# AlgoLab/rs-vgaligner

Measured on AMD Instinct MI355X. Metric: aligned reads/sec (10 kbp ONT vs HLA graph), higher is better.
Workload: dtype int32+f64

## Files before the change

### rs-vgaligner_amd/binding.py

```python
from __future__ import annotations

import ctypes as C
import os
from typing import List, Optional, Sequence

import numpy as np

_HERE = os.path.dirname(os.path.abspath(__file__))
LIB_PATH = os.environ.get("VGA_LIB") or os.path.join(_HERE, "libvga_hip.so")

VGA_OK = 0
VGA_MAX_KMER_LENGTH = 32
VGA_STRANDS_FORWARD = 0
VGA_STRANDS_BOTH = 1
ERR_NAMES = {-1: "VGA_ERR_ARG", -2: "VGA_ERR_HIP", -3: "VGA_ERR_NOMEM", -4: "VGA_ERR_UNSUPPORTED",
             -5: "VGA_ERR_NO_INDEX", -6: "VGA_ERR_NO_DEVICE", -7: "VGA_ERR_POOL"}

PILEUP_COLUMNS = ("A", "C", "G", "T", "N", "del", "ins")

ABI_SYMBOLS = [
    "vga_ctx_create", "vga_ctx_destroy", "vga_last_error", "vga_ctx_synchronize", "vga_abi_version",
    "vga_index_upload", "vga_batch_create", "vga_batch_destroy", "vga_batch_strands", "vga_map_default_params", "vga_map_batch",
    "vga_map_result_free", "vga_poa_default_params", "vga_poa_result_free", "vga_poa_batch", "vga_align_batch",
    "vga_align_result_free", "vga_last_kernel_times", "vga_chain_paths_text", "vga_chain_text_free",
    "vga_align_prepare", "vga_ctx_set_pool_fraction", "vga_ctx_set_host_threads",
    "vga_index_build_kmers", "vga_index_kmers_free",
    "vga_coverage_begin", "vga_coverage_read", "vga_coverage_reset", "vga_coverage_end",
    "vga_path_support_begin", "vga_path_support_read", "vga_path_support_last", "vga_path_support_reset", "vga_path_support_end",
    "vga_path_support_lists",
    "vga_pileup_begin", "vga_pileup_read", "vga_pileup_reset", "vga_pileup_end",
    "vga_genotype_begin", "vga_genotype_read", "vga_genotype_reset", "vga_genotype_end", "vga_genotype_pairs",
    "vga_genotype_lik_table", "vga_genotype_lik_begin", "vga_genotype_lik_read", "vga_genotype_lik_reset", "vga_genotype_lik_end",
    "vga_genotype_lik_pairs", "vga_genotype_lik_source",
    "vga_path_edit_begin", "vga_path_edit_read", "vga_path_edit_last", "vga_path_edit_reset", "vga_path_edit_end", "vga_path_edit_pairs",
    "vga_variant_call", "vga_variant_call_table",
    "vga_insertion_begin", "vga_insertion_read", "vga_insertion_reset", "vga_insertion_end", "vga_insertion_call", "vga_insertion_call_table",
    "vga_phase_begin", "vga_phase_read", "vga_phase_reset", "vga_phase_end", "vga_phase_links", "vga_phase_links_lists", "vga_phase_chain",
    "vga_phase_tags", "vga_phase_tags_lists",
    "vga_haplotype_counts", "vga_haplotype_counts_lists", "vga_haplotype_jobs", "vga_haplotype_call",
# ... 171 lines not shown
def load_library():
    global _lib
    if _lib is not None:
        return _lib
    if not os.path.exists(LIB_PATH):
        raise RuntimeError(f"{LIB_PATH} is missing: build it with `python -c 'import __graft_entry__ as g; g.build()'` "
                           "(there is no CPU fallback)")
    L = C.CDLL(LIB_PATH)
    vp = C.c_void_p
    L.vga_ctx_create.argtypes = [C.c_int, _P(vp)]
    L.vga_ctx_destroy.argtypes = [vp]
    L.vga_last_error.argtypes = [vp]
    L.vga_last_error.restype = C.c_char_p
    L.vga_ctx_synchronize.argtypes = [vp]
    L.vga_index_upload.argtypes = [vp, _P(IndexDesc)]
    L.vga_batch_create.argtypes = [vp, C.c_char_p, _P(C.c_uint64), C.c_uint64, _P(vp)]
    L.vga_batch_destroy.argtypes = [vp]
    if hasattr(L, "vga_batch_strands"):
        L.vga_batch_strands.argtypes = [vp, C.c_int, _P(C.c_char), _P(C.c_char)]
        L.vga_batch_strands.restype = C.c_int
    L.vga_map_default_params.argtypes = [_P(MapParams)]
    L.vga_map_batch.argtypes = [vp, _P(MapParams), _P(_P(MapResult))]
    L.vga_map_result_free.argtypes = [_P(MapResult)]
    L.vga_poa_default_params.argtypes = [_P(PoaParams)]
    L.vga_poa_result_free.argtypes = [_P(PoaResult)]
    L.vga_poa_batch.argtypes = [vp, C.c_uint64, _P(C.c_uint64), _P(C.c_uint64), C.c_char_p, _P(C.c_uint64),
                                _P(C.c_uint32), _P(C.c_uint32), _P(C.c_uint64), C.c_char_p, _P(PoaParams),
                                _P(_P(PoaResult))]
    L.vga_align_batch.argtypes = [vp, _P(MapResult), C.c_uint32, _P(PoaParams), _P(_P(AlignResult))]
    L.vga_align_result_free.argtypes = [_P(AlignResult)]
    L.vga_last_kernel_times.argtypes = [vp, _P(KernelTime), C.c_int]
    L.vga_chain_paths_text.argtypes = [vp, _P(MapResult), _P(_P(ChainText))]
    L.vga_align_prepare.argtypes = [vp, C.c_uint64, C.c_uint32]
    L.vga_align_prepare.restype = C.c_int
    L.vga_ctx_set_pool_fraction.argtypes = [vp, C.c_double]
    L.vga_ctx_set_pool_fraction.restype = C.c_int
    L.vga_ctx_set_host_threads.argtypes = [vp, C.c_uint32]
    L.vga_ctx_set_host_threads.restype = C.c_int
    L.vga_chain_text_free.argtypes = [_P(ChainText)]
    L.vga_index_build_kmers.argtypes = [vp, _P(IndexDesc), C.c_uint64, C.c_uint64]
    L.vga_index_build_kmers.restype = C.c_int
    L.vga_index_kmers_free.argtypes = [_P(IndexDesc)]
    L.vga_index_kmers_free.restype = None
    if hasattr(L, "vga_coverage_begin"):
        for name in ("vga_coverage_begin", "vga_coverage_reset", "vga_coverage_end"):
            getattr(L, name).argtypes = [vp]
# ... 305 lines not shown
        self.anchor_off = _np(r.anchor_off, R + 1, np.uint64)
        self.anchor_id = _np(r.anchor_id, A, np.uint32) if r.anchor_id else None
        self.query_begin = _np(r.query_begin, A, np.uint32)
        self.target_begin = _np(r.target_begin, A, np.uint32)
        self.target_end = _np(r.target_end, A, np.uint32)
        self.max_chain_score = _np(r.max_chain_score, A, np.float64) if r.max_chain_score else None
        self.best_pred_id = _np(r.best_pred_id, A, np.int32) if r.best_pred_id else None
        self.curr_max = _np(r.curr_max, R, np.float64)
        self.chain_off = _np(r.chain_off, R + 1, np.uint64)
        self.chain_placeholder = _np(r.chain_placeholder, nc, np.uint8)
        self.chain_anchor_off = _np(r.chain_anchor_off, nc + 1, np.uint64)
        self.chain_anchor_idx = _np(r.chain_anchor_idx, int(self.chain_anchor_off[-1]) if nc else 0, np.uint32)
        self.ms = {"probe": r.ms_probe, "sort": r.ms_sort, "chain": r.ms_chain, "total": r.ms_total}
        self.n_hits = int(r.n_hits)
        self.strand = _np(r.strand, R, np.uint8) if r.strand else None

    def chains_of(self, read: int):
        out = []
        for c in range(int(self.chain_off[read]), int(self.chain_off[read + 1])):
            s, e = int(self.chain_anchor_off[c]), int(self.chain_anchor_off[c + 1])
            out.append((bool(self.chain_placeholder[c]), self.chain_anchor_idx[s:e].tolist()))
        return out

    def close(self):
        if self._ptr is not None:
            self._L.vga_map_result_free(self._ptr)
            self._ptr = None

    def __del__(self):
        try:
            self.close()
        except Exception:
            pass


class PoaOut:
    def __init__(self, L, ptr):
        r = ptr.contents
        n = int(r.n)
        self.n = n
        self.ok = _np(r.ok, n, np.uint8)
        self.best_score = _np(r.best_score, n, np.int32)
        self.path_off = _np(r.path_off, n + 1, np.uint64)
        tp = int(self.path_off[-1])
        self.abpoa_nodes = _np(r.abpoa_nodes, tp, np.uint32)
        self.graph_nodes = _np(r.graph_nodes, tp, np.uint32)
        self.aln_start_offset = _np(r.aln_start_offset, n, np.uint32)
        self.aln_end_offset = _np(r.aln_end_offset, n, np.uint32)
        self.n_aligned_bases = _np(r.n_aligned_bases, n, np.uint32)
# ... 766 lines not shown
```

### rs-vgaligner_amd/csrc/vga_align.hip

```cpp
#include "vga_align_plan.hpp"
#include "vga_common.hpp"
#include "vga_coverage.hpp"
#include "vga_path_edit.hpp"
#include "vga_path_support.hpp"
#include "vga_pileup.hpp"
#include "vga_insertion.hpp"
#include "vga_poa_internal.hpp"
#include "vga_subgraph_host.hpp"

#include <algorithm>
#include <atomic>
#include <chrono>
#include <memory>

extern "C" void vga_align_result_free(vga_align_result *r)
{
    if (!r) return;
    free(r->aligned); free(r->path_off); free(r->path_handles); free(r->path_length); free(r->path_start);
    free(r->path_end); free(r->block_length); free(r->best_score); free(r->cigar_off); free(r->cigar);
    free(r->cs_off); free(r->cs);
    free(r);
}

namespace {
// ... 55 lines not shown
    if (m->strand)
        for (uint64_t r = 0; r < R && !any_rev; r++) any_rev = m->strand[r] != 0;
    if (!any_rev) return VGA_OK;
    const int rc = vga_batch_revcomp_device(b);
    if (rc != VGA_OK) return rc;
    vga_batch_revcomp_host(b);
    tr.mark("reverse complement");
    return VGA_OK;
}

int align_call::plan()
{
    const char *refused = nullptr;
    for (const oplist_maker *mk : oplist_makers()) {
        if (on_device || refused) break;
        refused = mk->counting(ctx) ? mk->text.refusal : mk == &cov_maker() && ps ? OPLIST_REFUSAL_PATHS : nullptr;
    }
    if (refused) return vga_set_error(ctx, VGA_ERR_UNSUPPORTED, OPLIST_ERR_REFUSED, refused);
    align_select(m, align_best_n, prob_read, prob_chain, read_prob0);
    n = prob_read.size();
    proxy.resize(n);
    west.resize(n);
    descs.resize(n);
    std::atomic<int> has_reverse{0};
    vga_parallel_for(n, [&](uint64_t p) {
        const align_prob a = align_plan_problem(m, prob_read[p], prob_chain[p], qlen(prob_read[p]), ctx->index.k, sw);
        proxy[p] = a.proxy; west[p] = a.west; descs[p] = a.desc;
        if (a.reverse) has_reverse = 1;
    });
    std::vector<uint32_t> ord(n);
    std::iota(ord.begin(), ord.end(), 0u);
    if (on_device) {
        ord = align_launch_order(proxy);
        align_permute(prob_read, ord); align_permute(prob_chain, ord); align_permute(proxy, ord); align_permute(west, ord); align_permute(descs, ord);
    }
    slot_of = align_slot_of(ord);
    if (has_reverse)
        return vga_set_error(ctx, VGA_ERR_UNSUPPORTED,
                             "a chain to be aligned holds reverse-strand anchors: RangeOrient::Reverse / Both (src/align.rs:365-387) is not supported");
    feed.views.resize(n);
    q_src.resize(on_device ? n : 0);
    for (uint64_t p = 0; p < n; p++) {
        const uint64_t r = prob_read[p];
        feed.views[p] = {nullptr, nullptr, 0, nullptr, nullptr, 0, b->reads.data() + q_off(r), qlen(r)};
        if (on_device) q_src[p] = q_off(r);
    }
    feed.proxy = proxy.data();
    return VGA_OK;
}

int align_call::device_store()
{
// ... 235 lines not shown
```

### rs-vgaligner_amd/csrc/vga_align_plan.hpp

```cpp
#pragma once

#include <algorithm>
#include <cmath>
#include <cstdint>
#include <cstdlib>
#include <cstring>
#include <numeric>
#include <vector>

#include "../../include/vga_hip.h"
#include "vga_sg_records.hpp"

struct align_switches {
    bool sg_host = false;
    uint32_t giant_rows = 24000u;
    double giant_cells = 1.5e8;
    bool has_sg_split = false;
    long sg_split = 0;
    bool trace = false;
};

static inline align_switches align_read_switches()
{
    align_switches s;
    if (const char *e = getenv("VGA_SUBGRAPH")) s.sg_host = strstr(e, "host") != nullptr;
    if (const char *e = getenv("VGA_GIANT_ROWS")) s.giant_rows = (uint32_t)atol(e);
    if (const char *e = getenv("VGA_GIANT_CELLS")) s.giant_cells = atof(e);
    if (const char *e = getenv("VGA_SG_SPLIT")) { s.has_sg_split = true; s.sg_split = atol(e); }
    if (const char *e = getenv("VGA_TRACE")) s.trace = atoi(e) != 0;
    return s;
}

static inline void align_select(const vga_map_result *m, uint32_t best_n, std::vector<uint64_t> &prob_read, std::vector<uint64_t> &prob_chain,
                                std::vector<uint64_t> &read_prob0)
{
    const uint64_t R = m->n_reads;
    prob_read.clear();
    prob_chain.clear();
    read_prob0.assign(R + 1, 0);
    for (uint64_t r = 0; r < R; r++) {
        read_prob0[r] = prob_read.size();
        const uint64_t c0 = m->chain_off[r], c1 = m->chain_off[r + 1];
        const uint64_t take = std::min<uint64_t>(best_n, c1 - c0);
        for (uint64_t c = c0; c < c0 + take; c++)
            if (!m->chain_placeholder[c]) { prob_read.push_back(r); prob_chain.push_back(c); }
    }
    read_prob0[R] = prob_read.size();
}

struct align_prob {
    sg_desc desc;
    uint32_t lo, hi;
    float west;
    double proxy;
    bool reverse;
};

static inline align_prob align_plan_problem(const vga_map_result *m, uint64_t r, uint64_t c, uint32_t qlen, uint32_t k, const align_switches &sw)
{
    align_prob o = {};
    const uint64_t a0 = m->anchor_off[r];
    const uint64_t c0 = m->chain_anchor_off[c], c1 = m->chain_anchor_off[c + 1];
    uint32_t lo = 0xFFFFFFFFu, hi = 0, pmin = 0xFFFFFFFFu, pmax = 0;
    for (uint64_t t = c0; t < c1; t++) {
        const uint64_t ai = a0 + m->chain_anchor_idx[t];
        lo = std::min(lo, m->target_begin[ai]);
        hi = std::max(hi, m->target_end[ai]);
        if ((m->target_begin[ai] | m->target_end[ai]) >> 31) o.reverse = true;
        const uint32_t s = m->target_begin[ai], e = m->target_end[ai] - 1;
        pmin = std::min(pmin, std::min(s, e));
        pmax = std::max(pmax, std::max(s, e));
    }
    o.lo = lo;
    o.hi = hi;
    const double q_first = c1 > c0 ? (double)m->query_begin[a0 + m->chain_anchor_idx[c0]] : 0.0;
    const double q_last = c1 > c0 ? (double)m->query_begin[a0 + m->chain_anchor_idx[c1 - 1]] + (double)k : (double)qlen;
    const double uncovered = q_first + std::max(0.0, (double)qlen - q_last);
    const double rows = (double)(hi > lo ? hi - lo : 0) + 1.6 * uncovered;
    o.west = (float)(650.0 + 0.3 * std::max(0.0, 0.85 * rows - (double)qlen));
    o.proxy = rows * (double)o.west;
    if (rows >= 0.85 * (double)sw.giant_rows) o.proxy += 1e13;
    if (c1 > c0) {
        const uint64_t fa = a0 + m->chain_anchor_idx[c0], la = a0 + m->chain_anchor_idx[c1 - 1];
        o.desc = {pmin, pmax, m->query_begin[fa], m->target_begin[fa], m->query_begin[la], m->target_end[la], qlen, 0u};
    }
    return o;
}

static inline std::vector<uint32_t> align_launch_order(const std::vector<double> &proxy)
{
    std::vector<uint32_t> ord(proxy.size());
    std::iota(ord.begin(), ord.end(), 0u);
    std::stable_sort(ord.begin(), ord.end(), [&](uint32_t x, uint32_t y) { return proxy[x] > proxy[y]; });
    return ord;
}

static inline std::vector<uint32_t> align_slot_of(const std::vector<uint32_t> &ord)
{
    std::vector<uint32_t> slot_of(ord.size());
    for (size_t i = 0; i < ord.size(); i++) slot_of[ord[i]] = (uint32_t)i;
    return slot_of;
}

template <typename T>
static inline void align_permute(std::vector<T> &v, const std::vector<uint32_t> &ord)
{
    std::vector<T> w(v.size());
    for (size_t i = 0; i < ord.size(); i++) w[i] = v[ord[i]];
    v.swap(w);
// ... 23 lines not shown
```

### rs-vgaligner_amd/csrc/vga_common.hpp

```cpp
#pragma once

#include <hip/hip_runtime.h>
#include <sys/mman.h>

#include <chrono>
#include <cstdarg>
#include <cstdint>
#include <cstdio>
#include <cstdlib>
#include <cstring>
#include <atomic>
#include <memory>
#include <mutex>
#include <new>
#include <string>
#include <thread>
#include <vector>

#include "../../include/vga_hip.h"
#include "vga_probe_hash.hpp"

#define VGA_ABI_VERSION 6

template <typename T>
using vga_owned = std::unique_ptr<T, void (*)(T *)>;
template <typename T, typename U = T>
vga_owned<T> vga_make_owned()
{
    return vga_owned<T>(new (std::nothrow) U(), [](T *p) { delete static_cast<U *>(p); });
}

struct cov_state;
struct ps_state;
struct pu_state;
struct ia_state;
struct ph_state;
struct poa_ws;

struct vga_dev_index {
    uint32_t k = 0;
    uint64_t seq_length = 0;
    uint64_t n_nodes = 0, n_edges = 0;
    uint32_t *d_table = nullptr;
// ... 38 lines not shown
    double pool_fraction = 1.0;
    unsigned host_threads = 0;
    std::mutex deferred_mu;
    std::vector<vga_deferred> deferred;
    std::atomic<int> alloc_urgent{0};
    vga_dev_index index;
    std::vector<vga_timer_entry> timers;
    std::vector<hipEvent_t> event_pool;
    size_t events_used = 0;
    struct agg_t {
        std::string name;
        float ms;
        uint32_t launches;
        uint64_t bytes;
        float busy_ms;
    };
    std::vector<agg_t> last_times;
    int n_cu = 256;
    vga_owned<void> map_ws{nullptr, nullptr};
    vga_owned<struct poa_ws> poa_ws{nullptr, nullptr};
    vga_owned<void> sg_ws{nullptr, nullptr};
    vga_owned<void> gaf_ws{nullptr, nullptr};
    std::vector<struct vga_batch *> batches;
};

struct vga_batch {
    vga_ctx *ctx = nullptr;
    int device = 0;
    uint64_t n_reads = 0;
    uint64_t total_bases = 0;
    std::vector<uint64_t> read_off;
    std::vector<char> reads;
    char *d_reads = nullptr;
    uint64_t *d_read_off = nullptr;
    bool rc_dev = false, rc_host = false;
    uint64_t *d_read_off2 = nullptr;
};
int vga_batch_revcomp_device(vga_batch *b);
void vga_batch_revcomp_host(vga_batch *b);

int vga_set_error(vga_ctx *ctx, int code, const char *fmt, ...);
void vga_index_release(vga_dev_index &ix);
int vga_index_load_graph(vga_ctx *ctx, const vga_index_desc *d);

#define VGA_HIP_CHECK(ctx, call)                                                               \
    do {                                                                                       \
        hipError_t e_ = (call);                                                                \
// ... 173 lines not shown
```

### rs-vgaligner_amd/csrc/vga_ctx.hip

```cpp
#include "vga_common.hpp"

#include <mutex>

#include <algorithm>

#include <malloc.h>

int vga_set_error(vga_ctx *ctx, int code, const char *fmt, ...)
{
    char buf[1024];
    va_list ap;
    va_start(ap, fmt);
    vsnprintf(buf, sizeof buf, fmt, ap);
    va_end(ap);
    if (ctx) { std::lock_guard<std::mutex> lk(ctx->err_mu); ctx->err = buf; }
    return code;
}

unsigned vga_host_threads(uint64_t n)
{
    unsigned nt = std::thread::hardware_concurrency();
    if (nt == 0) nt = 4;
    if (nt > 32) nt = 32;
    const char *e = getenv("VGA_HOST_THREADS");
// ... 25 lines not shown
void vga_defer_release(void *device_ptr, void *pinned_ptr, void *registered_ptr, size_t registered_bytes)
{
    const vga_deferred d = {device_ptr, pinned_ptr, registered_ptr, registered_bytes};
    vga_ctx *ctx = t_current_ctx;
    if (!ctx) { release_one(d); return; }
    std::lock_guard<std::mutex> lk(ctx->deferred_mu);
    ctx->deferred.push_back(d);
}

void vga_release_deferred(vga_ctx *ctx)
{
    if (!ctx) return;
    std::vector<vga_deferred> todo;
    {
        std::lock_guard<std::mutex> lk(ctx->deferred_mu);
        todo.swap(ctx->deferred);
    }
    if (todo.empty()) return;
    int cur = 0;
    (void)hipGetDevice(&cur);
    if (cur != ctx->device) (void)hipSetDevice(ctx->device);
    for (const vga_deferred &d : todo) release_one(d);
    if (cur != ctx->device) (void)hipSetDevice(cur);
}

extern "C" int vga_ctx_set_pool_fraction(vga_ctx *ctx, double fraction)
{
    if (!ctx) return VGA_ERR_ARG;
    if (!(fraction > 0.0) || fraction > 1.0) return vga_set_error(ctx, VGA_ERR_ARG, "vga_ctx_set_pool_fraction: %g is not in (0, 1]", fraction);
    ctx->pool_fraction = fraction;
    return VGA_OK;
}

extern "C" int vga_ctx_set_host_threads(vga_ctx *ctx, uint32_t n_threads)
{
    if (!ctx) return VGA_ERR_ARG;
    if (n_threads > 1024) return vga_set_error(ctx, VGA_ERR_ARG, "vga_ctx_set_host_threads: %u threads", n_threads);
    ctx->host_threads = n_threads;
    return VGA_OK;
}

extern "C" const char *vga_last_error(const vga_ctx *ctx)
{
    if (!ctx) return "null ctx";
    static thread_local std::string copy;
    {
// ... 45 lines not shown
    ix.cov.reset();
    ix.ps.reset();
    ix.pu.reset();
    ix.ia.reset();
    ix.ph.reset();
    ix = vga_dev_index();
}

extern "C" void vga_ctx_destroy(vga_ctx *ctx)
{
    if (!ctx) return;
    (void)hipSetDevice(ctx->device);
    vga_ctx_scope scope(ctx);
    if (ctx->stream) (void)hipStreamSynchronize(ctx->stream);
    for (vga_batch *b : ctx->batches) {
        if (b->d_reads) (void)hipFree(b->d_reads);
        if (b->d_read_off) (void)hipFree(b->d_read_off);
        if (b->d_read_off2) (void)hipFree(b->d_read_off2);
        b->d_reads = nullptr;
        b->d_read_off = nullptr;
        b->d_read_off2 = nullptr;
        b->ctx = nullptr;
    }
    ctx->map_ws.reset();
    ctx->poa_ws.reset();
    ctx->sg_ws.reset();
    ctx->gaf_ws.reset();
    vga_index_release(ctx->index);
    for (hipEvent_t ev : ctx->event_pool) (void)hipEventDestroy(ev);
    if (ctx->stream) (void)hipStreamDestroy(ctx->stream);
    vga_release_deferred(ctx);
    delete ctx;
}

extern "C" int vga_ctx_synchronize(vga_ctx *ctx)
{
    if (!ctx) return VGA_ERR_ARG;
    VGA_HIP_CHECK(ctx, hipStreamSynchronize(ctx->stream));
    return VGA_OK;
}

static hipEvent_t vga_event_get(vga_ctx *ctx)
{
    if (ctx->events_used == ctx->event_pool.size()) {
        hipEvent_t ev;
        if (hipEventCreate(&ev) != hipSuccess) return nullptr;
// ... 426 lines not shown
```

### rs-vgaligner_amd/csrc/vga_map.hip

```cpp
#include "vga_common.hpp"

#include <algorithm>
#include <chrono>
#include <cmath>
#include <memory>

#define VGA_WAVE 64
#define VGA_PROBE_NT 256
#define VGA_SORT_NT 256
#define VGA_NONE32 0xFFFFFFFFu

__device__ __forceinline__ uint32_t vga_lane() { return threadIdx.x & 63u; }

__device__ __forceinline__ uint32_t vga_wave_incl_scan(uint32_t v)
{
    uint32_t lane = vga_lane();
#pragma unroll
    for (int d = 1; d < 64; d <<= 1) {
        uint32_t o = __shfl_up(v, d, 64);
        if (lane >= (uint32_t)d) v += o;
    }
    return v;
}

// ... 444 lines not shown
        g_qb[o + i] = s_qb[a0 + i];
        g_tb[o + i] = s_tb[a0 + i];
        g_te[o + i] = s_te[a0 + i];
    }
    if (g_id)
        for (uint32_t i = threadIdx.x; i < A; i += blockDim.x) {
            g_id[o + i] = s_id[a0 + i];
            g_f[o + i] = f[a0 + i];
            g_pred[o + i] = pred[a0 + i];
        }
}

__global__ __launch_bounds__(256) void k_chain_compact_sel(const uint32_t *__restrict__ sel, const uint64_t *__restrict__ anchor_off,
                                                           const uint32_t *__restrict__ sel_chain_words, const uint64_t *__restrict__ woff,
                                                           const uint32_t *__restrict__ chain_buf, uint32_t *__restrict__ comp)
{
    const uint64_t r = blockIdx.x, s = sel[r];
    const uint32_t *src = chain_buf + 3 * anchor_off[s] + 2 * s;
    uint32_t *dst = comp + woff[r];
    const uint32_t n = sel_chain_words[r];
    for (uint32_t i = threadIdx.x; i < n; i += blockDim.x) dst[i] = src[i];
}

namespace {

struct map_ws {
    vga_dbuf<uint32_t> cnt;
    vga_dbuf<uint64_t> anchor_off;
    vga_dbuf<uint32_t> a_qb, a_tb, a_te, a_idx, key_b, val_b, s_qb, s_tb, s_te;
    vga_dbuf<double> f, curr_max, gap_cost;
    vga_dbuf<int32_t> pred_id, pred_pos;
    vga_dbuf<uint32_t> chain_buf, chain_cnt, chain_words, key_a, chain_comp;
    vga_dbuf<uint64_t> chain_woff;
    vga_dbuf<uint8_t> strand;
    vga_dbuf<uint32_t> sel, sel_anchors, sel_chain_cnt, sel_chain_words, g_qb, g_tb, g_te, g_id;
    vga_dbuf<uint64_t> sel_off;
    vga_dbuf<double> sel_curr_max, g_f;
    vga_dbuf<int32_t> g_pred;
    vga_hbuf<uint64_t> h_chain_woff;
    vga_hbuf<uint32_t> h_chain_cnt, h_chain_words, h_cnt;
    vga_hbuf<double> h_curr_max;
    hipStream_t st_copy = nullptr;
    hipEvent_t ev_sorted = nullptr;
    ~map_ws()
    {
        if (st_copy) (void)hipStreamDestroy(st_copy);
        if (ev_sorted) (void)hipEventDestroy(ev_sorted);
    }
};

}

extern "C" void vga_map_result_free(vga_map_result *r)
{
    if (!r) return;
    free(r->anchor_off);
    free(r->anchor_id);
    free(r->query_begin);
    free(r->target_begin);
    free(r->target_end);
    free(r->max_chain_score);
    free(r->best_pred_id);
    free(r->curr_max);
    free(r->chain_off);
    free(r->chain_placeholder);
    free(r->chain_anchor_off);
    free(r->chain_anchor_idx);
    free(r->strand);
    free(r);
}

namespace {

struct map_source {
    const double *curr_max = nullptr;
    const uint32_t *chain_cnt = nullptr, *chain_words = nullptr;
    const uint32_t *ids = nullptr;
    const double *f = nullptr;
// ... 2 lines not shown

struct map_call {
    vga_ctx *const ctx;
    vga_batch *const b;
    const vga_map_params *const params;
    const vga_dev_index &ix;
    const uint64_t R;
    const bool all_orients;
    const bool both;
    const uint64_t RV;
    const bool emit_dp;
    const hipStream_t st;
    map_ws &ws;
    const std::chrono::steady_clock::time_point t_host0 = std::chrono::steady_clock::now();
    vga_trace tr{"map"};
    const uint64_t *d_read_off = nullptr;
    std::vector<uint64_t> aoff_v;
    uint64_t total = 0;
    std::vector<double> gc;
    const uint32_t *perm = nullptr;
    int t_total = -1;
    map_source src;
    uint64_t chain_total_words = 0;
    std::unique_ptr<uint32_t, void (*)(void *)> chain_words_host{nullptr, free};
    vga_result_guard<vga_map_result, vga_map_result_free> res;

    map_call(vga_batch *batch, const vga_map_params *p, map_ws &w)
        : ctx(batch->ctx), b(batch), params(p), ix(batch->ctx->index), R(batch->n_reads), all_orients(!p->only_forward),
          both(p->strands == VGA_STRANDS_BOTH), RV(both ? 2 * R : R), emit_dp(p->emit_dp != 0), st(batch->ctx->stream), ws(w)
    {
        res.wait[0] = &st;
        res.wait[1] = &ws.st_copy;
    }

    int nomem() { return vga_set_error(ctx, VGA_ERR_NOMEM, "out of host memory (map result of %llu reads)", (unsigned long long)R); }
    bool alloc_anchor_arrays(size_t n);
    int begin_result();
    template <bool EMIT>
    void launch_probe();
    int count();
    int emit_and_sort();
    template <bool GAP_LDS>
    void launch_chain(size_t lds_bytes, uint32_t key_anchors);
    void chain();
    int source_forward();
    int source_picked();
// ... 158 lines not shown
        launch_chain<false>(0, key_anchors);
    vga_timer_end(ctx, t4);
    vga_timer_end(ctx, t_total);
    tr.mark("chain launch");
}

bool map_call::alloc_anchor_arrays(size_t n)
{
    if (emit_dp) {
        res->anchor_id = xmalloc<uint32_t>(n);
        res->max_chain_score = xmalloc<double>(n);
        res->best_pred_id = xmalloc<int32_t>(n);
    }
    res->query_begin = xmalloc<uint32_t>(n);
    res->target_begin = xmalloc<uint32_t>(n);
    res->target_end = xmalloc<uint32_t>(n);
    return !((emit_dp && (!res->anchor_id || !res->max_chain_score || !res->best_pred_id)) || !res->query_begin || !res->target_begin ||
             !res->target_end);
}

int map_call::source_forward()
{
    src = {ws.curr_max.p, ws.chain_cnt.p, ws.chain_words.p, perm, ws.f.p, ws.pred_id.p};
    const size_t An = (size_t)total;
    if (!alloc_anchor_arrays(An)) return nomem();
    if (An) {
        VGA_HIP_CHECK(ctx, hipMemcpyAsync(res->query_begin, ws.s_qb.p, An * 4, hipMemcpyDeviceToHost, ws.st_copy));
        VGA_HIP_CHECK(ctx, hipMemcpyAsync(res->target_begin, ws.s_tb.p, An * 4, hipMemcpyDeviceToHost, ws.st_copy));
        VGA_HIP_CHECK(ctx, hipMemcpyAsync(res->target_end, ws.s_te.p, An * 4, hipMemcpyDeviceToHost, ws.st_copy));
    }
    return VGA_OK;
}

int map_call::source_picked()
{
    VGA_HIP_CHECK(ctx, ws.strand.reserve(R)); VGA_HIP_CHECK(ctx, ws.sel.reserve(R)); VGA_HIP_CHECK(ctx, ws.sel_anchors.reserve(R));
    VGA_HIP_CHECK(ctx, ws.sel_curr_max.reserve(R)); VGA_HIP_CHECK(ctx, ws.sel_chain_cnt.reserve(R)); VGA_HIP_CHECK(ctx, ws.sel_chain_words.reserve(R));
    VGA_HIP_CHECK(ctx, ws.sel_off.reserve(R + 1));
    const int tp = vga_timer_begin(ctx, "strand_pick", 2 * R * (8 + 8 + 4 + 4) + R * (1 + 4 + 4 + 8 + 4 + 4) + R * (4 + 8));
    hipLaunchKernelGGL(k_strand_pick, dim3((unsigned)((R + 255) / 256)), dim3(256), 0, st, (uint32_t)R, ws.anchor_off.p, ws.curr_max.p,
                       ws.chain_cnt.p, ws.chain_words.p, ws.strand.p, ws.sel.p, ws.sel_anchors.p, ws.sel_curr_max.p, ws.sel_chain_cnt.p,
                       ws.sel_chain_words.p);
    hipLaunchKernelGGL(k_strand_scan, dim3(1), dim3(256), 0, st, (uint32_t)R, ws.sel_anchors.p, ws.sel_off.p);
    vga_timer_end(ctx, tp);
    VGA_HIP_CHECK(ctx, hipMemcpyAsync(res->anchor_off, ws.sel_off.p, (R + 1) * 8, hipMemcpyDeviceToHost, st));
    VGA_HIP_CHECK(ctx, hipMemcpyAsync(res->strand, ws.strand.p, R, hipMemcpyDeviceToHost, st));
// ... 11 lines not shown
    VGA_HIP_CHECK(ctx, hipMemcpyAsync(ws.h_chain_cnt.p, src.chain_cnt, R * 4, hipMemcpyDeviceToHost, st));
    VGA_HIP_CHECK(ctx, hipMemcpyAsync(ws.h_chain_words.p, src.chain_words, R * 4, hipMemcpyDeviceToHost, st));
    VGA_HIP_CHECK(ctx, hipStreamSynchronize(st));
    return VGA_OK;
}

int map_call::gather_picked()
{
    const size_t As = (size_t)res->anchor_off[R];
    res->n_anchors = As;
    if (!alloc_anchor_arrays(As)) return nomem();
    VGA_HIP_CHECK(ctx, ws.g_qb.reserve(As)); VGA_HIP_CHECK(ctx, ws.g_tb.reserve(As)); VGA_HIP_CHECK(ctx, ws.g_te.reserve(As));
    if (emit_dp) { VGA_HIP_CHECK(ctx, ws.g_id.reserve(As)); VGA_HIP_CHECK(ctx, ws.g_f.reserve(As)); VGA_HIP_CHECK(ctx, ws.g_pred.reserve(As)); }
    const int tg = vga_timer_begin(ctx, "strand_gather", (uint64_t)As * 2 * (12 + (emit_dp ? 16 : 0)) + R * 20);
    hipLaunchKernelGGL(k_strand_gather, dim3((unsigned)R), dim3(256), 0, st, ws.sel.p, ws.anchor_off.p, ws.sel_off.p, ws.s_qb.p, ws.s_tb.p,
                       ws.s_te.p, perm, ws.f.p, ws.pred_id.p, ws.g_qb.p, ws.g_tb.p, ws.g_te.p, emit_dp ? ws.g_id.p : nullptr,
                       emit_dp ? ws.g_f.p : nullptr, emit_dp ? ws.g_pred.p : nullptr);
    vga_timer_end(ctx, tg);
    if (As) {
        VGA_HIP_CHECK(ctx, hipMemcpyAsync(res->query_begin, ws.g_qb.p, As * 4, hipMemcpyDeviceToHost, st));
        VGA_HIP_CHECK(ctx, hipMemcpyAsync(res->target_begin, ws.g_tb.p, As * 4, hipMemcpyDeviceToHost, st));
        VGA_HIP_CHECK(ctx, hipMemcpyAsync(res->target_end, ws.g_te.p, As * 4, hipMemcpyDeviceToHost, st));
    }
    src.ids = ws.g_id.p;
    src.f = ws.g_f.p;
    src.pred = ws.g_pred.p;
    return VGA_OK;
}

int map_call::fetch_chains()
{
    const size_t An_res = (size_t)res->n_anchors;
    for (uint64_t r = 0; r < R; r++) { ws.h_chain_woff.p[r] = chain_total_words; chain_total_words += ws.h_chain_words.p[r]; }
    ws.h_chain_woff.p[R] = chain_total_words;
    chain_words_host.reset(xmalloc<uint32_t>(chain_total_words + 2));
    if (!chain_words_host) return nomem();
    if (chain_total_words) {
        VGA_HIP_CHECK(ctx, ws.chain_comp.reserve(chain_total_words + 2));
        VGA_HIP_CHECK(ctx, hipMemcpyAsync(ws.chain_woff.p, ws.h_chain_woff.p, (R + 1) * 8, hipMemcpyHostToDevice, st));
        if (both)
            hipLaunchKernelGGL(k_chain_compact_sel, dim3((unsigned)R), dim3(256), 0, st, ws.sel.p, ws.anchor_off.p, ws.sel_chain_words.p,
                               ws.chain_woff.p, ws.chain_buf.p, ws.chain_comp.p);
        else
            hipLaunchKernelGGL(k_chain_compact, dim3((unsigned)R), dim3(256), 0, st, ws.anchor_off.p, ws.chain_words.p, ws.chain_woff.p,
                               ws.chain_buf.p, ws.chain_comp.p);
        VGA_HIP_CHECK(ctx, hipMemcpyAsync(chain_words_host.get(), ws.chain_comp.p, chain_total_words * 4, hipMemcpyDeviceToHost, st));
    }
    if (An_res && emit_dp) {
        VGA_HIP_CHECK(ctx, hipMemcpyAsync(res->anchor_id, src.ids, An_res * 4, hipMemcpyDeviceToHost, st));
        VGA_HIP_CHECK(ctx, hipMemcpyAsync(res->max_chain_score, src.f, An_res * 8, hipMemcpyDeviceToHost, st));
        VGA_HIP_CHECK(ctx, hipMemcpyAsync(res->best_pred_id, src.pred, An_res * 4, hipMemcpyDeviceToHost, st));
    }
    VGA_HIP_CHECK(ctx, hipStreamSynchronize(st));
    VGA_HIP_CHECK(ctx, hipStreamSynchronize(ws.st_copy));
    tr.mark("kernels + D2H");
    vga_timers_collect(ctx);
    memcpy(res->curr_max, ws.h_curr_max.p, R * 8);
    return VGA_OK;
}

int map_call::assemble()
{
    const uint32_t *h_chain_cnt = ws.h_chain_cnt.p, *h_chain_words = ws.h_chain_words.p, *h_chain_buf = chain_words_host.get();
    uint64_t n_chains = 0, n_members = 0;
    std::vector<uint64_t> mem0(R);
    for (uint64_t r = 0; r < R; r++) {
        uint32_t c = h_chain_cnt[r];
        res->chain_off[r] = n_chains;
        mem0[r] = n_members;
        n_chains += c ? c : 1;
        n_members += h_chain_words[r] - c;
    }
    res->chain_off[R] = n_chains;
    res->n_chains = n_chains;
    res->chain_placeholder = xmalloc<uint8_t>(n_chains);
    res->chain_anchor_off = xmalloc<uint64_t>(n_chains + 1);
    res->chain_anchor_idx = xmalloc<uint32_t>(n_members);
    if (!res->chain_placeholder || !res->chain_anchor_off || !res->chain_anchor_idx) return nomem();
    res->chain_anchor_off[n_chains] = n_members;
    vga_map_result *const out = res.p;
    vga_parallel_for(R, [&](uint64_t r) {
        uint64_t ci = out->chain_off[r], mi = mem0[r];
        const uint32_t *buf = h_chain_buf + ws.h_chain_woff.p[r];
        uint32_t c = h_chain_cnt[r], wp = 0;
        if (c == 0) {
            out->chain_placeholder[ci] = 1;
            out->chain_anchor_off[ci] = mi;
            return;
        }
        for (uint32_t q = 0; q < c; q++) {
            uint32_t len = buf[wp++];
            out->chain_placeholder[ci] = 0;
            out->chain_anchor_off[ci] = mi;
// ... 16 lines not shown
static int vga_map_batch_impl(vga_batch *b, const vga_map_params *params, vga_map_result **out)
{
    if (!b || !params || !out || !b->ctx) return VGA_ERR_ARG;
    vga_ctx *ctx = b->ctx;
    *out = nullptr;
    (void)hipSetDevice(ctx->device);
    vga_ctx_scope scope(ctx);
    vga_release_deferred(ctx);
    int rc = map_validate(ctx, params);
    if (rc != VGA_OK) return rc;
    if (!ctx->map_ws && !(ctx->map_ws = vga_make_owned<void, map_ws>())) throw std::bad_alloc();
    vga_timers_reset(ctx);
    map_call c(b, params, *(map_ws *)ctx->map_ws.get());
    if ((rc = c.begin_result()) != VGA_OK) return rc;
    if (c.R > 0) {
        if ((rc = c.count()) != VGA_OK) return rc;
        if ((rc = c.emit_and_sort()) != VGA_OK) return rc;
        c.chain();
        if ((rc = c.both ? c.source_picked() : c.source_forward()) != VGA_OK) return rc;
        if ((rc = c.fetch_counts()) != VGA_OK) return rc;
        if (c.both && (rc = c.gather_picked()) != VGA_OK) return rc;
        if ((rc = c.fetch_chains()) != VGA_OK) return rc;
        if ((rc = c.assemble()) != VGA_OK) return rc;
    }
    *out = c.res.release();
    return VGA_OK;
}

extern "C" int vga_map_batch(vga_batch *b, const vga_map_params *params, vga_map_result **out)
{
    try {
        return vga_map_batch_impl(b, params, out);
    } catch (const std::bad_alloc &) {
        return vga_set_error((b ? b->ctx : nullptr), VGA_ERR_NOMEM, "vga_map_batch: out of host memory");
    } catch (const std::exception &e) {
        return vga_set_error((b ? b->ctx : nullptr), VGA_ERR_ARG, "vga_map_batch: %s", e.what());
    }
}
```

### rs-vgaligner_amd/csrc/vga_sg_records.hpp

```cpp
#pragma once

#include <cstdint>

struct sg_desc {
    uint32_t pmin, pmax;
    uint32_t q_first, t_first;
    uint32_t q_last, te_last;
    uint32_t qlen, pad;
};

struct sg_sum {
    uint32_t n_nodes;
    uint32_t N;
    uint32_t n_preds, n_sinks;
    uint32_t wlo, whi;
    uint32_t longest;
    uint32_t life;
    uint32_t flags;
    uint32_t pad[3];
};

struct sg_off {
    uint64_t node0;
    uint64_t pred0, sink0, seq0;
    uint64_t q_src;
};
```

Measured before the change: 10650.

## Compute per-chain summaries on GPU during mapping and reuse them for align planning

Adds a GPU kernel that reduces each chain's anchors into a summary record (span, min/max positions, first/last anchor coordinates, strand flag) at the end of the map call. The records are copied back and cached per map result in the context. The align planner then reads these instead of scanning the anchors on the host, which removes a parallel host pass from align setup. The cost is an extra kernel, an extra device-to-host copy, a global mutex-protected registry keyed by result pointer, and the planning loop now runs serially.

```diff
diff --git a/rs-vgaligner_amd/binding.py b/rs-vgaligner_amd/binding.py
--- a/rs-vgaligner_amd/binding.py
+++ b/rs-vgaligner_amd/binding.py
@@ -15,6 +15,8 @@
 VGA_STRANDS_BOTH = 1
 ERR_NAMES = {-1: "VGA_ERR_ARG", -2: "VGA_ERR_HIP", -3: "VGA_ERR_NOMEM", -4: "VGA_ERR_UNSUPPORTED",
              -5: "VGA_ERR_NO_INDEX", -6: "VGA_ERR_NO_DEVICE", -7: "VGA_ERR_POOL"}
+
+CHAIN_SUMMARY_FIELDS = ("lo", "hi", "pmin", "pmax", "q_first", "t_first", "q_last", "te_last", "n_anchors", "reverse")
 
 PILEUP_COLUMNS = ("A", "C", "G", "T", "N", "del", "ins")
 
@@ -232,6 +234,8 @@
     L.vga_map_default_params.argtypes = [_P(MapParams)]
     L.vga_map_batch.argtypes = [vp, _P(MapParams), _P(_P(MapResult))]
     L.vga_map_result_free.argtypes = [_P(MapResult)]
+    if hasattr(L, "vga_debug_chain_summary"):
+        L.vga_debug_chain_summary.argtypes = [vp, _P(MapResult), C.c_uint64, _P(C.c_uint32)]
     L.vga_poa_default_params.argtypes = [_P(PoaParams)]
     L.vga_poa_result_free.argtypes = [_P(PoaResult)]
     L.vga_poa_batch.argtypes = [vp, C.c_uint64, _P(C.c_uint64), _P(C.c_uint64), C.c_char_p, _P(C.c_uint64),
@@ -583,9 +587,36 @@
             out.append((bool(self.chain_placeholder[c]), self.chain_anchor_idx[s:e].tolist()))
         return out
 
+    def chain_summaries(self, ctx: "Context"):
+        out = np.zeros((self.n_chains, len(CHAIN_SUMMARY_FIELDS)), dtype=np.uint32)
+        row = np.zeros(len(CHAIN_SUMMARY_FIELDS), dtype=np.uint32)
+        for c in range(self.n_chains):
+            ctx._check(self._L.vga_debug_chain_summary(ctx.h, self._ptr, c, _u32p(row)))
+            out[c] = row
+        return out
+
+    def detached(self) -> "MapOut":
+        src, keep, dst = self._ptr.contents, [], MapResult()
+        sizes = dict(anchor_off=self.n_reads + 1, anchor_id=self.n_anchors, query_begin=self.n_anchors, target_begin=self.n_anchors,
+                     target_end=self.n_anchors, max_chain_score=self.n_anchors, best_pred_id=self.n_anchors, curr_max=self.n_reads,
+                     chain_off=self.n_reads + 1, chain_placeholder=self.n_chains, chain_anchor_off=self.n_chains + 1,
+                     chain_anchor_idx=len(self.chain_anchor_idx), strand=self.n_reads)
+        for name, typ in MapResult._fields_:
+            v = getattr(src, name)
+            if name in sizes and v:
+                buf = (typ._type_ * max(1, sizes[name]))()
+                C.memmove(buf, v, sizes[name] * C.sizeof(typ._type_))
+                keep.append(buf)
+                v = C.cast(buf, typ)
+            setattr(dst, name, v)
+        copy = MapOut(self._L, C.pointer(dst))
+        copy._keep, copy._owned = keep, False
+        return copy
+
     def close(self):
         if self._ptr is not None:
-            self._L.vga_map_result_free(self._ptr)
+            if getattr(self, "_owned", True):
+                self._L.vga_map_result_free(self._ptr)
             self._ptr = None
 
     def __del__(self):
diff --git a/rs-vgaligner_amd/csrc/vga_align.hip b/rs-vgaligner_amd/csrc/vga_align.hip
--- a/rs-vgaligner_amd/csrc/vga_align.hip
+++ b/rs-vgaligner_amd/csrc/vga_align.hip
@@ -101,12 +101,21 @@
     proxy.resize(n);
     west.resize(n);
     descs.resize(n);
+    const chain_summaries known = sw.plan_host ? nullptr : vga_summaries_of(ctx, m);
+    const bool summarised = known && known->size() == m->n_chains;
+    if (sw.trace) fprintf(stderr, "[vga-trace] align: plan from %s\n", summarised ? "the map call's chain summaries" : "a host pass over the anchors");
     std::atomic<int> has_reverse{0};
-    vga_parallel_for(n, [&](uint64_t p) {
-        const align_prob a = align_plan_problem(m, prob_read[p], prob_chain[p], qlen(prob_read[p]), ctx->index.k, sw);
+    const auto plan_one = [&](uint64_t p) {
+        const uint32_t ql = qlen(prob_read[p]);
+        const align_prob a = summarised ? align_plan_from_summary((*known)[prob_chain[p]], ql, ctx->index.k, sw)
+                                        : align_plan_problem(m, prob_read[p], prob_chain[p], ql, ctx->index.k, sw);
         proxy[p] = a.proxy; west[p] = a.west; descs[p] = a.desc;
         if (a.reverse) has_reverse = 1;
-    });
+    };
+    if (summarised)
+        for (uint64_t p = 0; p < n; p++) plan_one(p);
+    else
+        vga_parallel_for(n, plan_one);
     std::vector<uint32_t> ord(n);
     std::iota(ord.begin(), ord.end(), 0u);
     if (on_device) {
diff --git a/rs-vgaligner_amd/csrc/vga_align_plan.hpp b/rs-vgaligner_amd/csrc/vga_align_plan.hpp
--- a/rs-vgaligner_amd/csrc/vga_align_plan.hpp
+++ b/rs-vgaligner_amd/csrc/vga_align_plan.hpp
@@ -18,6 +18,7 @@
     bool has_sg_split = false;
     long sg_split = 0;
     bool trace = false;
+    bool plan_host = false;
 };
 
 static inline align_switches align_read_switches()
@@ -28,6 +29,7 @@
     if (const char *e = getenv("VGA_GIANT_CELLS")) s.giant_cells = atof(e);
     if (const char *e = getenv("VGA_SG_SPLIT")) { s.has_sg_split = true; s.sg_split = atol(e); }
     if (const char *e = getenv("VGA_TRACE")) s.trace = atoi(e) != 0;
+    if (const char *e = getenv("VGA_ALIGN_PLAN")) s.plan_host = strstr(e, "host") != nullptr;
     return s;
 }
 
@@ -56,35 +58,51 @@
     bool reverse;
 };
 
-static inline align_prob align_plan_problem(const vga_map_result *m, uint64_t r, uint64_t c, uint32_t qlen, uint32_t k, const align_switches &sw)
+static inline chain_summary align_chain_summary(const vga_map_result *m, uint64_t r, uint64_t c)
+{
+    chain_summary s = {0xFFFFFFFFu, 0u, 0xFFFFFFFFu, 0u, 0u, 0u, 0u, 0u, 0u, 0u};
+    const uint64_t a0 = m->anchor_off[r];
+    const uint64_t c0 = m->chain_anchor_off[c], c1 = m->chain_anchor_off[c + 1];
+    for (uint64_t t = c0; t < c1; t++) {
+        const uint64_t ai = a0 + m->chain_anchor_idx[t];
+        s.lo = std::min(s.lo, m->target_begin[ai]);
+        s.hi = std::max(s.hi, m->target_end[ai]);
+        if ((m->target_begin[ai] | m->target_end[ai]) >> 31) s.reverse = 1;
+        const uint32_t b = m->target_begin[ai], e = m->target_end[ai] - 1;
+        s.pmin = std::min(s.pmin, std::min(b, e));
+        s.pmax = std::max(s.pmax, std::max(b, e));
+    }
+    s.n_anchors = (uint32_t)(c1 - c0);
+    if (c1 > c0) {
+        const uint64_t fa = a0 + m->chain_anchor_idx[c0], la = a0 + m->chain_anchor_idx[c1 - 1];
+        s.q_first = m->query_begin[fa]; s.t_first = m->target_begin[fa];
+        s.q_last = m->query_begin[la]; s.te_last = m->target_end[la];
+    }
+    return s;
+}
+
+static inline align_prob align_plan_from_summary(const chain_summary &s, uint32_t qlen, uint32_t k, const align_switches &sw)
 {
     align_prob o = {};
-    const uint64_t a0 = m->anchor_off[r];
-    const uint64_t c0 = m->chain_anchor_off[c], c1 = m->chain_anchor_off[c + 1];
-    uint32_t lo = 0xFFFFFFFFu, hi = 0, pmin = 0xFFFFFFFFu, pmax = 0;
-    for (uint64_t t = c0; t < c1; t++) {
-        const uint64_t ai = a0 + m->chain_anchor_idx[t];
-        lo = std::min(lo, m->target_begin[ai]);
-        hi = std::max(hi, m->target_end[ai]);
-        if ((m->target_begin[ai] | m->target_end[ai]) >> 31) o.reverse = true;
-        const uint32_t s = m->target_begin[ai], e = m->target_end[ai] - 1;
-        pmin = std::min(pmin, std::min(s, e));
-        pmax = std::max(pmax, std::max(s, e));
-    }
+    const uint32_t lo = s.lo, hi = s.hi;
+    const bool any = s.n_anchors > 0;
     o.lo = lo;
     o.hi = hi;
-    const double q_first = c1 > c0 ? (double)m->query_begin[a0 + m->chain_anchor_idx[c0]] : 0.0;
-    const double q_last = c1 > c0 ? (double)m->query_begin[a0 + m->chain_anchor_idx[c1 - 1]] + (double)k : (double)qlen;
+    o.reverse = s.reverse != 0;
+    const double q_first = any ? (double)s.q_first : 0.0;
+    const double q_last = any ? (double)s.q_last + (double)k : (double)qlen;
     const double uncovered = q_first + std::max(0.0, (double)qlen - q_last);
     const double rows = (double)(hi > lo ? hi - lo : 0) + 1.6 * uncovered;
     o.west = (float)(650.0 + 0.3 * std::max(0.0, 0.85 * rows - (double)qlen));
     o.proxy = rows * (double)o.west;
     if (rows >= 0.85 * (double)sw.giant_rows) o.proxy += 1e13;
-    if (c1 > c0) {
-        const uint64_t fa = a0 + m->chain_anchor_idx[c0], la = a0 + m->chain_anchor_idx[c1 - 1];
-        o.desc = {pmin, pmax, m->query_begin[fa], m->target_begin[fa], m->query_begin[la], m->target_end[la], qlen, 0u};
-    }
+    if (any) o.desc = {s.pmin, s.pmax, s.q_first, s.t_first, s.q_last, s.te_last, qlen, 0u};
     return o;
+}
+
+static inline align_prob align_plan_problem(const vga_map_result *m, uint64_t r, uint64_t c, uint32_t qlen, uint32_t k, const align_switches &sw)
+{
+    return align_plan_from_summary(align_chain_summary(m, r, c), qlen, k, sw);
 }
 
 static inline std::vector<uint32_t> align_launch_order(const std::vector<double> &proxy)
diff --git a/rs-vgaligner_amd/csrc/vga_common.hpp b/rs-vgaligner_amd/csrc/vga_common.hpp
--- a/rs-vgaligner_amd/csrc/vga_common.hpp
+++ b/rs-vgaligner_amd/csrc/vga_common.hpp
@@ -15,10 +15,12 @@
 #include <new>
 #include <string>
 #include <thread>
+#include <unordered_map>
 #include <vector>
 
 #include "../../include/vga_hip.h"
 #include "vga_probe_hash.hpp"
+#include "vga_sg_records.hpp"
 
 #define VGA_ABI_VERSION 6
 
@@ -103,7 +105,14 @@
     vga_owned<void> sg_ws{nullptr, nullptr};
     vga_owned<void> gaf_ws{nullptr, nullptr};
     std::vector<struct vga_batch *> batches;
-};
+    std::unordered_map<const vga_map_result *, std::shared_ptr<const std::vector<chain_summary>>> summaries;
+};
+
+using chain_summaries = std::shared_ptr<const std::vector<chain_summary>>;
+void vga_summaries_put(vga_ctx *ctx, const vga_map_result *m, std::vector<chain_summary> &&recs);
+chain_summaries vga_summaries_of(vga_ctx *ctx, const vga_map_result *m);
+void vga_summaries_drop(const vga_map_result *m);
+void vga_summaries_drop_all(vga_ctx *ctx);
 
 struct vga_batch {
     vga_ctx *ctx = nullptr;
diff --git a/rs-vgaligner_amd/csrc/vga_ctx.hip b/rs-vgaligner_amd/csrc/vga_ctx.hip
--- a/rs-vgaligner_amd/csrc/vga_ctx.hip
+++ b/rs-vgaligner_amd/csrc/vga_ctx.hip
@@ -71,6 +71,44 @@
     if (cur != ctx->device) (void)hipSetDevice(ctx->device);
     for (const vga_deferred &d : todo) release_one(d);
     if (cur != ctx->device) (void)hipSetDevice(cur);
+}
+
+namespace {
+std::mutex g_summaries_mu;
+std::unordered_map<const vga_map_result *, vga_ctx *> g_summaries_owner;
+}
+
+void vga_summaries_put(vga_ctx *ctx, const vga_map_result *m, std::vector<chain_summary> &&recs)
+{
+    auto held = std::make_shared<const std::vector<chain_summary>>(std::move(recs));
+    std::lock_guard<std::mutex> lk(g_summaries_mu);
+    const auto it = g_summaries_owner.find(m);
+    if (it != g_summaries_owner.end() && it->second != ctx) it->second->summaries.erase(m);
+    g_summaries_owner[m] = ctx;
+    ctx->summaries[m] = std::move(held);
+}
+
+chain_summaries vga_summaries_of(vga_ctx *ctx, const vga_map_result *m)
+{
+    std::lock_guard<std::mutex> lk(g_summaries_mu);
+    const auto it = ctx->summaries.find(m);
+    return it == ctx->summaries.end() ? nullptr : it->second;
+}
+
+void vga_summaries_drop(const vga_map_result *m)
+{
+    std::lock_guard<std::mutex> lk(g_summaries_mu);
+    const auto it = g_summaries_owner.find(m);
+    if (it == g_summaries_owner.end()) return;
+    it->second->summaries.erase(m);
+    g_summaries_owner.erase(it);
+}
+
+void vga_summaries_drop_all(vga_ctx *ctx)
+{
+    std::lock_guard<std::mutex> lk(g_summaries_mu);
+    for (const auto &e : ctx->summaries) g_summaries_owner.erase(e.first);
+    ctx->summaries.clear();
 }
 
 extern "C" int vga_ctx_set_pool_fraction(vga_ctx *ctx, double fraction)
@@ -162,6 +200,7 @@
         b->d_read_off2 = nullptr;
         b->ctx = nullptr;
     }
+    vga_summaries_drop_all(ctx);
     ctx->map_ws.reset();
     ctx->poa_ws.reset();
     ctx->sg_ws.reset();
diff --git a/rs-vgaligner_amd/csrc/vga_map.hip b/rs-vgaligner_amd/csrc/vga_map.hip
--- a/rs-vgaligner_amd/csrc/vga_map.hip
+++ b/rs-vgaligner_amd/csrc/vga_map.hip
@@ -490,6 +490,60 @@
     for (uint32_t i = threadIdx.x; i < n; i += blockDim.x) dst[i] = src[i];
 }
 
+__global__ __launch_bounds__(256) void k_chain_summary(const uint64_t *__restrict__ off, const uint32_t *__restrict__ chain_cnt,
+                                                       const uint32_t *__restrict__ chain_words, const uint64_t *__restrict__ woff,
+                                                       const uint64_t *__restrict__ chain_off, const uint32_t *__restrict__ comp,
+                                                       const uint32_t *__restrict__ qb, const uint32_t *__restrict__ tb,
+                                                       const uint32_t *__restrict__ te, chain_summary *__restrict__ out)
+{
+    const uint64_t r = blockIdx.x;
+    const uint32_t lane = threadIdx.x & 63u, wave = threadIdx.x >> 6;
+    const uint32_t c = chain_cnt[r], n = chain_words[r];
+    chain_summary *const rec = out + chain_off[r];
+    if (c == 0) {
+        if (threadIdx.x == 0) rec[0] = {0xFFFFFFFFu, 0u, 0xFFFFFFFFu, 0u, 0u, 0u, 0u, 0u, 0u, 0u};
+        return;
+    }
+    const uint64_t a0 = off[r];
+    const uint32_t A = (uint32_t)(off[r + 1] - a0);
+    const uint32_t *const buf = comp + woff[r];
+    uint32_t wp = 0;
+    for (uint32_t q = 0; q < c && wp < n; q++) {
+        const uint32_t len = buf[wp];
+        const uint32_t *const mem = buf + wp + 1;
+        wp += 1 + len;
+        if (wp > n) break;
+        if ((q & 3u) != wave) continue;
+        uint32_t lo = 0xFFFFFFFFu, hi = 0, pmin = 0xFFFFFFFFu, pmax = 0, rev = 0;
+        for (uint32_t t = lane; t < len; t += 64) {
+            const uint32_t i = mem[t];
+            if (i >= A) continue;
+            const uint32_t b = tb[a0 + i], e1 = te[a0 + i], e = e1 - 1u;
+            lo = min(lo, b);
+            hi = max(hi, e1);
+            rev |= (b | e1) >> 31;
+            pmin = min(pmin, min(b, e));
+            pmax = max(pmax, max(b, e));
+        }
+        for (int d = 32; d > 0; d >>= 1) {
+            lo = min(lo, (uint32_t)__shfl_xor((int)lo, d, 64));
+            hi = max(hi, (uint32_t)__shfl_xor((int)hi, d, 64));
+            pmin = min(pmin, (uint32_t)__shfl_xor((int)pmin, d, 64));
+            pmax = max(pmax, (uint32_t)__shfl_xor((int)pmax, d, 64));
+            rev |= (uint32_t)__shfl_xor((int)rev, d, 64);
+        }
+        if (lane == 0) {
+            chain_summary s = {lo, hi, pmin, pmax, 0u, 0u, 0u, 0u, len, rev};
+            if (len > 0) {
+                const uint32_t fa = mem[len - 1], la = mem[0];
+                if (fa < A) { s.q_first = qb[a0 + fa]; s.t_first = tb[a0 + fa]; }
+                if (la < A) { s.q_last = qb[a0 + la]; s.te_last = te[a0 + la]; }
+            }
+            rec[q] = s;
+        }
+    }
+}
+
 namespace {
 
 struct map_ws {
@@ -508,6 +562,10 @@
     vga_hbuf<uint64_t> h_chain_woff;
     vga_hbuf<uint32_t> h_chain_cnt, h_chain_words, h_cnt;
     vga_hbuf<double> h_curr_max;
+    vga_dbuf<uint64_t> chain_off;
+    vga_hbuf<uint64_t> h_chain_off;
+    vga_dbuf<chain_summary> summ;
+    vga_hbuf<chain_summary> h_summ;
     hipStream_t st_copy = nullptr;
     hipEvent_t ev_sorted = nullptr;
     ~map_ws()
@@ -522,6 +580,7 @@
 extern "C" void vga_map_result_free(vga_map_result *r)
 {
     if (!r) return;
+    vga_summaries_drop(r);
     free(r->anchor_off);
     free(r->anchor_id);
     free(r->query_begin);
@@ -570,6 +629,10 @@
     int t_total = -1;
     map_source src;
     uint64_t chain_total_words = 0;
+    uint64_t n_chains = 0;
+    const uint64_t *res_off = nullptr;
+    const uint32_t *res_qb = nullptr, *res_tb = nullptr, *res_te = nullptr;
+    std::vector<chain_summary> summaries;
     std::unique_ptr<uint32_t, void (*)(void *)> chain_words_host{nullptr, free};
     vga_result_guard<vga_map_result, vga_map_result_free> res;
 
@@ -774,6 +837,7 @@
 int map_call::source_forward()
 {
     src = {ws.curr_max.p, ws.chain_cnt.p, ws.chain_words.p, perm, ws.f.p, ws.pred_id.p};
+    res_off = ws.anchor_off.p; res_qb = ws.s_qb.p; res_tb = ws.s_tb.p; res_te = ws.s_te.p;
     const size_t An = (size_t)total;
     if (!alloc_anchor_arrays(An)) return nomem();
     if (An) {
@@ -831,6 +895,7 @@
         VGA_HIP_CHECK(ctx, hipMemcpyAsync(res->target_begin, ws.g_tb.p, As * 4, hipMemcpyDeviceToHost, st));
         VGA_HIP_CHECK(ctx, hipMemcpyAsync(res->target_end, ws.g_te.p, As * 4, hipMemcpyDeviceToHost, st));
     }
+    res_off = ws.sel_off.p; res_qb = ws.g_qb.p; res_tb = ws.g_tb.p; res_te = ws.g_te.p;
     src.ids = ws.g_id.p;
     src.f = ws.g_f.p;
     src.pred = ws.g_pred.p;
@@ -840,13 +905,20 @@
 int map_call::fetch_chains()
 {
     const size_t An_res = (size_t)res->n_anchors;
-    for (uint64_t r = 0; r < R; r++) { ws.h_chain_woff.p[r] = chain_total_words; chain_total_words += ws.h_chain_words.p[r]; }
+    VGA_HIP_CHECK(ctx, ws.h_chain_off.reserve(R + 1)); VGA_HIP_CHECK(ctx, ws.chain_off.reserve(R + 1));
+    for (uint64_t r = 0; r < R; r++) {
+        ws.h_chain_woff.p[r] = chain_total_words; chain_total_words += ws.h_chain_words.p[r];
+        ws.h_chain_off.p[r] = n_chains; n_chains += ws.h_chain_cnt.p[r] ? ws.h_chain_cnt.p[r] : 1;
+    }
     ws.h_chain_woff.p[R] = chain_total_words;
+    ws.h_chain_off.p[R] = n_chains;
     chain_words_host.reset(xmalloc<uint32_t>(chain_total_words + 2));
     if (!chain_words_host) return nomem();
+    VGA_HIP_CHECK(ctx, ws.chain_comp.reserve(chain_total_words + 2));
+    VGA_HIP_CHECK(ctx, ws.summ.reserve(n_chains)); VGA_HIP_CHECK(ctx, ws.h_summ.reserve(n_chains));
+    VGA_HIP_CHECK(ctx, hipMemcpyAsync(ws.chain_woff.p, ws.h_chain_woff.p, (R + 1) * 8, hipMemcpyHostToDevice, st));
+    VGA_HIP_CHECK(ctx, hipMemcpyAsync(ws.chain_off.p, ws.h_chain_off.p, (R + 1) * 8, hipMemcpyHostToDevice, st));
     if (chain_total_words) {
-        VGA_HIP_CHECK(ctx, ws.chain_comp.reserve(chain_total_words + 2));
-        VGA_HIP_CHECK(ctx, hipMemcpyAsync(ws.chain_woff.p, ws.h_chain_woff.p, (R + 1) * 8, hipMemcpyHostToDevice, st));
         if (both)
             hipLaunchKernelGGL(k_chain_compact_sel, dim3((unsigned)R), dim3(256), 0, st, ws.sel.p, ws.anchor_off.p, ws.sel_chain_words.p,
                                ws.chain_woff.p, ws.chain_buf.p, ws.chain_comp.p);
@@ -855,6 +927,9 @@
                                ws.chain_buf.p, ws.chain_comp.p);
         VGA_HIP_CHECK(ctx, hipMemcpyAsync(chain_words_host.get(), ws.chain_comp.p, chain_total_words * 4, hipMemcpyDeviceToHost, st));
     }
+    VGA_HIP_CHECK(ctx, vga_launch_on(ctx, st, "chain_summary", chain_total_words * (4 + 8) + n_chains * sizeof(chain_summary) + R * 32, k_chain_summary, dim3((unsigned)R), dim3(256), res_off, src.chain_cnt, src.chain_words, ws.chain_woff.p,
+                                     ws.chain_off.p, ws.chain_comp.p, res_qb, res_tb, res_te, ws.summ.p));
+    VGA_HIP_CHECK(ctx, hipMemcpyAsync(ws.h_summ.p, ws.summ.p, n_chains * sizeof(chain_summary), hipMemcpyDeviceToHost, st));
     if (An_res && emit_dp) {
         VGA_HIP_CHECK(ctx, hipMemcpyAsync(res->anchor_id, src.ids, An_res * 4, hipMemcpyDeviceToHost, st));
         VGA_HIP_CHECK(ctx, hipMemcpyAsync(res->max_chain_score, src.f, An_res * 8, hipMemcpyDeviceToHost, st));
@@ -865,19 +940,19 @@
     tr.mark("kernels + D2H");
     vga_timers_collect(ctx);
     memcpy(res->curr_max, ws.h_curr_max.p, R * 8);
+    summaries.assign(ws.h_summ.p, ws.h_summ.p + n_chains);
     return VGA_OK;
 }
 
 int map_call::assemble()
 {
     const uint32_t *h_chain_cnt = ws.h_chain_cnt.p, *h_chain_words = ws.h_chain_words.p, *h_chain_buf = chain_words_host.get();
-    uint64_t n_chains = 0, n_members = 0;
+    uint64_t n_members = 0;
     std::vector<uint64_t> mem0(R);
     for (uint64_t r = 0; r < R; r++) {
         uint32_t c = h_chain_cnt[r];
-        res->chain_off[r] = n_chains;
+        res->chain_off[r] = ws.h_chain_off.p[r];
         mem0[r] = n_members;
-        n_chains += c ? c : 1;
         n_members += h_chain_words[r] - c;
     }
     res->chain_off[R] = n_chains;
@@ -940,12 +1015,24 @@
         if (c.both && (rc = c.gather_picked()) != VGA_OK) return rc;
         if ((rc = c.fetch_chains()) != VGA_OK) return rc;
         if ((rc = c.assemble()) != VGA_OK) return rc;
+        vga_summaries_put(ctx, c.res.p, std::move(c.summaries));
     }
     *out = c.res.release();
     return VGA_OK;
 }
 
-extern "C" int vga_map_batch(vga_batch *b, const vga_map_params *params, vga_map_result **out)
+extern "C" int vga_debug_chain_summary(vga_ctx *ctx, const vga_map_result *m, uint64_t chain, uint32_t *out10)
+{
+    if (!ctx || !m || !out10) return VGA_ERR_ARG;
+    const chain_summaries s = vga_summaries_of(ctx, m);
+    if (!s) return vga_set_error(ctx, VGA_ERR_ARG, "vga_debug_chain_summary: not a live map result of this context");
+    if (chain >= s->size()) return vga_set_error(ctx, VGA_ERR_ARG, "vga_debug_chain_summary: chain %llu of %llu", (unsigned long long)chain, (unsigned long long)s->size());
+    static_assert(sizeof(chain_summary) == 10 * sizeof(uint32_t), "chain_summary is ten 32-bit fields");
+    memcpy(out10, &(*s)[chain], sizeof(chain_summary));
+    return VGA_OK;
+}
+
+extern "C" int vga_map_batch(vga_batch *b,const vga_map_params *params, vga_map_result **out)
 {
     try {
         return vga_map_batch_impl(b, params, out);
diff --git a/rs-vgaligner_amd/csrc/vga_sg_records.hpp b/rs-vgaligner_amd/csrc/vga_sg_records.hpp
--- a/rs-vgaligner_amd/csrc/vga_sg_records.hpp
+++ b/rs-vgaligner_amd/csrc/vga_sg_records.hpp
@@ -7,6 +7,15 @@
     uint32_t q_first, t_first;
     uint32_t q_last, te_last;
     uint32_t qlen, pad;
+};
+
+struct chain_summary {
+    uint32_t lo, hi;
+    uint32_t pmin, pmax;
+    uint32_t q_first, t_first;
+    uint32_t q_last, te_last;
+    uint32_t n_anchors;
+    uint32_t reverse;
 };
 
 struct sg_sum {
```

Result: no change. 10620 (-0.3%).
